# Unalome81/IEEE-802.11-OFDM-QPSK-Simulator

Measured on NVIDIA B200. Metric: OFDM symbols/s, TX+AWGN+RX chain (BER/EVM sweep), higher is better.
Workload: dtype f32+f64

## Files before the change

ieee-802.11-ofdm-qpsk-simulator_b200/csrc/ofdm_b200.cu:

```cuda
#include <cmath>
#include <cstdio>
#include <cstdlib>
#include <cstring>
#include <mutex>
#include <new>
#include <set>
#include <utility>

#include "ofdm_chain.cuh"
#include "ofdm_stream.cuh"
#include "ofdm_mc_quad.cuh"
#include "ofdm_sweep.cuh"

using namespace ofdm;

struct ofdm_ctx {
    int device = 0;
    int sm_count = 0;
    cudaStream_t stream = nullptr;
    bool owns_stream = false;
    cudaStream_t copy_stream = nullptr;
    cudaEvent_t copy_done[2] = {nullptr, nullptr}, call_start = nullptr;
    uint64_t launches = 0;
    bool force_generic = false;
// ... 21 lines not shown

const signed char kLk[53] = {1, 1, -1, -1, 1, 1, -1, 1, -1, 1, 1, 1, 1, 1, 1, -1, -1, 1, 1, -1, 1, -1, 1, 1, 1, 1, 0,
                             1, -1, -1, 1, 1, -1, 1, -1, 1, -1, -1, -1, -1, -1, 1, 1, -1, -1, 1, -1, 1, -1, 1, 1, 1, 1};

int fail(ofdm_ctx *ctx, int status, const char *what, cudaError_t e = cudaSuccess)
{
    if (ctx) {
        if (e != cudaSuccess) snprintf(ctx->err, sizeof ctx->err, "%s: %s", what, cudaGetErrorString(e));
        else snprintf(ctx->err, sizeof ctx->err, "%s", what);
    }
    return status;
}

#define OFDM_CUDA(ctx, call)                                                   \
    do {                                                                       \
        cudaError_t e_ = (call);                                               \
        if (e_ != cudaSuccess) return fail((ctx), OFDM_ERR_CUDA, #call, e_);   \
    } while (0)

#define OFDM_REQUIRE(ctx, cond)                                                          \
    do {                                                                                 \
        if (!(cond)) return fail((ctx), OFDM_ERR_INVALID, "invalid argument: " #cond);   \
    } while (0)

int check_launch(ofdm_ctx *ctx, const char *name)
{
    cudaError_t e = cudaGetLastError();
    if (e != cudaSuccess) return fail(ctx, OFDM_ERR_CUDA, name, e);
    ctx->launches += 1;
    return OFDM_OK;
}

int bind(ofdm_ctx *ctx)
{
    if (!ctx) return OFDM_ERR_INVALID;
    OFDM_CUDA(ctx, cudaSetDevice(ctx->device));
    return OFDM_OK;
}

template <typename K>
cudaError_t allow_smem(ofdm_ctx *ctx, K kernel, size_t bytes)
{
    static std::mutex mu;
    static std::set<std::pair<const void *, int>> done;
    std::lock_guard<std::mutex> lock(mu);
    const std::pair<const void *, int> key(reinterpret_cast<const void *>(kernel), ctx->device);
    if (done.count(key)) return cudaSuccess;
    const cudaError_t e = cudaFuncSetAttribute(kernel, cudaFuncAttributeMaxDynamicSharedMemorySize, (int)bytes);
    if (e == cudaSuccess) done.insert(key);
    return e;
}

template <typename K>
int grid_for(ofdm_ctx *ctx, K kernel, size_t dyn_smem, long work_items_per_block_iter, long work)
{
    int per_sm = 1;
    if (cudaOccupancyMaxActiveBlocksPerMultiprocessor(&per_sm, kernel, kThreads, dyn_smem) != cudaSuccess || per_sm < 1) per_sm = 1;
    long full = (long)per_sm * ctx->sm_count;
    long need = (work + work_items_per_block_iter - 1) / work_items_per_block_iter;
    long g = need < full ? need : full;
    return (int)(g < 1 ? 1 : g);
}

int stream_grid(ofdm_ctx *ctx, long rows, int rows_per_block, int per_sm)
{
    const long need = (rows + rows_per_block - 1) / rows_per_block, full = (long)per_sm * ctx->sm_count;
    const long g = need < full ? need : full;
    return (int)(g < 1 ? 1 : g);
}

int ensure_scratch(ofdm_ctx *ctx, int slot, size_t bytes, void **out)
{
    if (ctx->scratch_bytes[slot] < bytes) {
        if (ctx->scratch[slot]) { cudaFree(ctx->scratch[slot]); ctx->scratch[slot] = nullptr; ctx->scratch_bytes[slot] = 0; }
        cudaError_t e = cudaMalloc(&ctx->scratch[slot], bytes);
        if (e != cudaSuccess) return fail(ctx, OFDM_ERR_NOMEM, "cudaMalloc(scratch)", e);
        ctx->scratch_bytes[slot] = bytes;
    }
    *out = ctx->scratch[slot];
    return OFDM_OK;
}

float snr_linear(float snr_db)
{
    return (float)pow(10.0, (double)(snr_db / 10));
}

__global__ void k_power_prefix(const float2 *__restrict__ x, int n, float *__restrict__ out)
{
    float p = 0.f;
    for (int i = 0; i < n; ++i) {
        const double h = hypot_glibc((double)x[i].x, (double)x[i].y);
        p = __double2float_rn(__dadd_rn((double)p, __dmul_rn(h, h)));
    }
    *out = p;
}

struct DeviceTables {
    bool ready = false;
    float lts_freq[128], lts_time[320], sts_time[320], lts_power_prefix;
};
std::mutex g_tables_mutex;
DeviceTables g_tables[64];

int upload_tables(ofdm_ctx *ctx, const float *lts_time , float power_prefix)
{
    Tables t;
    memset(&t, 0, sizeof t);
    for (int k = 0; k < 32; ++k) t.tw64[k] = make_double2(kTw64[k][0], kTw64[k][1]);
    for (int k = 0; k < 64; ++k) {
// ... 783 lines not shown
    if (int st = ensure_scratch(ctx, 2, (size_t)n_frames * sizeof(float), &power)) return st;
    if (int st = ensure_scratch(ctx, 3, sizeof(ofdm_counters) * (size_t)n_snr, &cnt)) return st;
    if (!ctx->copy_stream) {
        OFDM_CUDA(ctx, cudaStreamCreateWithFlags(&ctx->copy_stream, cudaStreamNonBlocking));
        for (int i = 0; i < 2; ++i) OFDM_CUDA(ctx, cudaEventCreateWithFlags(&ctx->copy_done[i], cudaEventDisableTiming));
        OFDM_CUDA(ctx, cudaEventCreateWithFlags(&ctx->call_start, cudaEventDisableTiming));
    }
    OFDM_CUDA(ctx, cudaEventRecord(ctx->call_start, ctx->stream));
    OFDM_CUDA(ctx, cudaStreamWaitEvent(ctx->copy_stream, ctx->call_start, 0));
    OFDM_CUDA(ctx, cudaMemsetAsync(cnt, 0, sizeof(ofdm_counters) * (size_t)n_snr, ctx->stream));
    const long chunk = 65536;
    int c = 0;
    for (long f0 = 0; f0 < n_frames; f0 += chunk, ++c) {
        const long n = n_frames - f0 < chunk ? n_frames - f0 : chunk;
        char *db = (char *)bits + f0 * bits_per_frame, *dg = (char *)g + f0 * g_per_frame;
        OFDM_CUDA(ctx, cudaMemcpyAsync(db, (const char *)bits_host + f0 * bits_per_frame, n * bits_per_frame, cudaMemcpyHostToDevice, ctx->copy_stream));
        const char *hg = (const char *)g_host + f0 * g_per_frame;
        if (n_sym <= 4) {
            OFDM_CUDA(ctx, cudaMemcpy2DAsync(dg + 32 * 4, g_per_frame, hg + 32 * 4, g_per_frame, 128 * 4, n, cudaMemcpyHostToDevice, ctx->copy_stream));
            for (int sy = 0; sy < n_sym; ++sy) {
                const size_t off = (size_t)(160 + 80 * sy + 16) * 4;
                OFDM_CUDA(ctx, cudaMemcpy2DAsync(dg + off, g_per_frame, hg + off, g_per_frame, 64 * 4, n, cudaMemcpyHostToDevice, ctx->copy_stream));
            }
        } else {
            OFDM_CUDA(ctx, cudaMemcpyAsync(dg, hg, n * g_per_frame, cudaMemcpyHostToDevice, ctx->copy_stream));
        }
        OFDM_CUDA(ctx, cudaEventRecord(ctx->copy_done[c & 1], ctx->copy_stream));
        OFDM_CUDA(ctx, cudaStreamWaitEvent(ctx->stream, ctx->copy_done[c & 1], 0));
        float *fr = (float *)frames + f0 * len * 2, *pw = (float *)power + f0;
        if (int st = ofdm_tx_frames(ctx, (const uint32_t *)db, fr, pw, n, n_sym, mode)) return st;
        if (int st = sweep_points(ctx, fr, (const float *)dg, pw, (const uint32_t *)db, n, n_sym, snr_db, n_snr, mode,
                                  (ofdm_counters *)cnt))
            return st;
    }
    OFDM_CUDA(ctx, cudaMemcpyAsync(out_host, cnt, sizeof(ofdm_counters) * (size_t)n_snr, cudaMemcpyDeviceToHost, ctx->stream));
    OFDM_CUDA(ctx, cudaStreamSynchronize(ctx->stream));
    return OFDM_OK;
}

}

namespace {
int sweep_points(ofdm_ctx *ctx, const float *frames, const float *g, const float *power, const uint32_t *bits, long n_frames, int n_sym,
                 const float *snr_db, int n_snr, int mode, ofdm_counters *counters)
{
    const bool aligned = ((uintptr_t)frames % 16 == 0) && ((uintptr_t)g % 16 == 0);
    const bool fused = ctx->fused_sweep && n_sym == 2 && aligned && !ctx->force_generic && !ctx->general_stream &&
                       (mode != OFDM_MODE_EXACT || ctx->checked);
    if (!fused) {
        for (int i = 0; i < n_snr; ++i)
            if (int st = ofdm_awgn_rx_inject(ctx, frames, g, power, bits, snr_db[i], n_frames, n_sym, mode, counters + i, nullptr)) return st;
        return OFDM_OK;
    }
    const size_t smem = sweep_smem_bytes();
    const long max_frames = 1L << 30;
    for (int s0 = 0; s0 < n_snr; s0 += kMaxSnr) {
        SweepParams p;
        memset(&p, 0, sizeof p);
        p.n_snr = n_snr - s0 < kMaxSnr ? n_snr - s0 : kMaxSnr;
        for (int i = 0; i < p.n_snr; ++i) p.snr_lin[i] = snr_linear(snr_db[s0 + i]);
        p.radius_scale = ctx->force_replay ? INFINITY : kRadius;
        p.replayed = ctx->replayed_dev;
        p.evm_guard = ctx->evm_guard;
        p.counters = counters + s0;
        for (long f0 = 0; f0 < n_frames; f0 += max_frames) {
            p.n_frames = n_frames - f0 < max_frames ? n_frames - f0 : max_frames;
            p.in = reinterpret_cast<const float2 *>(frames) + f0 * 320;
            p.g = g + f0 * 320;
            p.power = power + f0;
            p.tx_bits = bits + f0 * 6;
            auto launch = [&](auto k) -> int {
                OFDM_CUDA(ctx, allow_smem(ctx, k, smem));
                int grid = grid_for(ctx, k, smem, kWarpsPerBlock, p.n_frames);
                k<<<grid, kThreads, smem, ctx->stream>>>(p);
                return check_launch(ctx, "k_sweep_lin");
            };
            if (int st = mode == OFDM_MODE_EXACT ? launch(k_sweep_lin<kArithChecked>) : launch(k_sweep_lin<kArithFast>)) return st;
        }
    }
    return OFDM_OK;
}
}

extern "C" {

int ofdm_random_bits(ofdm_ctx *ctx, uint32_t seed, uint64_t frame0, long n_frames, int n_sym, uint32_t *bits)
{
    if (int st = bind(ctx)) return st;
    OFDM_REQUIRE(ctx, n_frames >= 0 && nsym_ok(n_sym));
    if (n_frames == 0) return OFDM_OK;
    OFDM_REQUIRE(ctx, bits != nullptr);
    long n = n_frames * n_sym;
    k_philox_bits<<<blocks_1d(n), 256, 0, ctx->stream>>>(seed, frame0, n, n_sym, bits);
    return check_launch(ctx, "k_philox_bits");
}

}

namespace {
int mc_awgn_core(ofdm_ctx *ctx, uint32_t seed, uint64_t frame0, long n_frames, int n_sym, const float *snr_db, const uint32_t *streams,
                 int n_snr, int mode, ofdm_counters *counters)
{
    if (n_sym == 2) {
        const size_t smem = mc_smem_bytes();
        const long max_frames = 1L << 30;
        for (long f0 = 0; f0 < n_frames; f0 += max_frames) {
            McParams p;
            memset(&p, 0, sizeof p);
            p.seed = seed; p.frame0 = frame0 + (uint64_t)f0; p.n_frames = n_frames - f0 < max_frames ? n_frames - f0 : max_frames;
            p.n_snr = n_snr; p.counters = counters;
            for (int i = 0; i < n_snr; ++i) {
                p.snr_lin[i] = snr_linear(snr_db[i]); p.inv_sqrt_snr[i] = (float)(1.0 / sqrt((double)p.snr_lin[i]));
                p.stream[i] = streams ? streams[i] : (uint32_t)i;
            }
            p.radius_scale = ctx->force_replay ? INFINITY : kRadius;
            p.replayed = ctx->replayed_dev;
            p.evm_guard = ctx->evm_guard;
            p.radius_chan = ctx->force_replay ? INFINITY : kChanRadius * sqrtf(320.f) * 1.001f;
            auto launch = [&](auto k) -> int {
                OFDM_CUDA(ctx, allow_smem(ctx, k, smem));
                int grid = grid_for(ctx, k, smem, kWarpsPerBlock, p.n_frames);
                k<<<grid, kThreads, smem, ctx->stream>>>(p);
                return check_launch(ctx, "k_mc_philox");
            };
            auto launch_quad = [&](auto k) -> int {
                const size_t qsmem = mc_quad_smem_bytes();
                OFDM_CUDA(ctx, allow_smem(ctx, k, qsmem));
// ... 521 lines not shown
```

ieee-802.11-ofdm-qpsk-simulator_b200/csrc/ofdm_chain.cuh:

```cuda
#pragma once
#include "ofdm_kernels.cuh"

namespace ofdm {

constexpr int kWin = 72;
constexpr int kMaxSnr = 64;
constexpr int kMaxTaps = 16;

struct ItemConst {
    int f_off[3];
    int bin[3];
    float sc[3];
    int word[3];
    int shift[3];
};

__constant__ unsigned char c_deal_bin[48] = { 2, 10, 12, 14, 16, 23, 49, 54,    1,  3, 18, 40, 46, 60, 61, 63,   22, 25, 45, 47, 48, 50, 52, 59,
                                              4,  6,  9, 11, 13, 24, 39, 58,    8, 41, 42, 44, 51, 53, 55, 62,    5, 15, 17, 19, 20, 26, 38, 56};

__device__ __forceinline__ ItemConst make_items(int lane)
{
    ItemConst c;
#pragma unroll
    for (int r = 0; r < 3; ++r) {
        const int sym = (lane >> 3) & 1;
        const int bin = c_deal_bin[(2 * r + (lane >> 4)) * 8 + (lane & 7)];
        const int d = c_tab.bin_data[bin];
        c.f_off[r] = sym * kWin + bin;
        c.bin[r] = bin;
        c.sc[r] = 0.5f * (float)c_tab.bin_lts[bin];
        c.word[r] = sym * 3 + (d >> 4);
        c.shift[r] = 2 * (d & 15);
    }
    return c;
}

template <bool EXACT>
__device__ __forceinline__ uint32_t item_eval(float2 F, float2 Hh, float sc, uint32_t txp, float &e2)
{
    return process_bin_hot<EXACT>(F, Hh, sc, txp, true, e2);
}

enum { kArithFast = 0, kArithExact = 1, kArithChecked = 2 };
constexpr float kRadius = 320.f * 5.9604645e-8f;
constexpr float kChanRadius = 18.f * 5.9604645e-8f;


__device__ __forceinline__ float window_radius(float2 n2v, float scale, float extra)
{
    float n2 = n2v.x + n2v.y;
    n2 += __shfl_xor_sync(0xffffffffu, n2, 1);
    n2 += __shfl_xor_sync(0xffffffffu, n2, 2);
    n2 += __shfl_xor_sync(0xffffffffu, n2, 4);
    float r;
    asm("sqrt.approx.ftz.f32 %0, %1;" : "=f"(r) : "f"(n2));
    return (n2 >= 1e-30f && n2 < 1e20f) ? fmaf(scale, r, extra) : __int_as_float(0x7f800000);
}

constexpr float kEvmGuard = 820.f;
template <int LEVEL, bool THR_GIVEN = false>
__device__ __forceinline__ uint32_t process_bin_spec(float2 F, float2 G, float k, uint32_t txp, float rF, float rH2, float den_min4,
                                                     float2 &e2, bool &doubt)
{
    const float a = F.x, b = F.y, c = G.x, d = G.y;
    const float2 pt = __fmul2_rn(make_float2(d, d), make_float2(b, a));
    const float2 S = __ffma2_rn(make_float2(c, c), F, make_float2(pt.x, -pt.y));
    const float sr = S.x, si = S.y;
    const float den = fmaf(c, c, d * d);
    float inv;
    asm("rcp.approx.ftz.f32 %0, %1;" : "=f"(inv) : "f"(den));
    const uint32_t sq = txp << 31, sx = (txp ^ (txp >> 1)) << 31;
    const uint32_t kb = __float_as_uint(k);
    const uint32_t ei_ = (__float_as_uint(sr) ^ sx ^ kb) >> 31, eq_ = (__float_as_uint(si) ^ sq ^ kb) >> 31;
    bool safe;
    if (LEVEL >= 2) {
        float thr;
        if (THR_GIVEN) thr = rF;
        else {
            const float fa = fabsf(a) + fabsf(b), hc = fabsf(c) + fabsf(d);
            thr = fmaf(rF, hc + rH2, fmaf(rH2, fa, 1.2e-7f * (fa * hc)));
        }
        safe = (fminf(fabsf(sr), fabsf(si)) - thr) > 2e-30f && (THR_GIVEN || den < 1.6e14f) && den > den_min4;
    } else {
        safe = (THR_GIVEN || den < 1.6e14f) && den > den_min4;
    }
    doubt = doubt || !safe;
    const float2 U = __fmul2_rn(S, make_float2(inv, inv));
    const float2 D = __ffma2_rn(U, make_float2(k, k), make_float2(__uint_as_float(0xBF3504F3u ^ sx), __uint_as_float(0xBF3504F3u ^ sq)));
    e2 = __ffma2_rn(D, D, e2);
    return ei_ | (eq_ << 8) | ((ei_ & eq_) << 16);
}
__device__ __forceinline__ uint32_t process_bin_checked(float2 F, float2 G, float k, uint32_t txp, float rF, float rH2, float den_min4,
                                                        float2 &e2, bool &doubt)
{
    return process_bin_spec<2>(F, G, k, txp, rF, rH2, den_min4, e2, doubt);
}

struct McParams {
    uint32_t seed;
    uint64_t frame0;
    long n_frames;
    int n_snr;
    float snr_lin[kMaxSnr];
    float inv_sqrt_snr[kMaxSnr];
    uint32_t stream[kMaxSnr];
    float radius_scale;
    float radius_chan;
    float evm_guard;
    int n_taps;
    ofdm_counters *counters;
    unsigned long long *replayed;
};

struct WarpShared {
    float2 tile[kWarpTile];
    float2 lts[2][kWin];
    float2 body[2][kWin];
    uint2 res[kMaxSnr];
};

__device__ __noinline__ uint2 mc_point_replay(const float2 *src, double sigma_d, uint32_t seed, uint32_t stream, uint64_t fr,
                                              uint32_t txp3, float2 *ws_tile, float2 *ws_lts, unsigned long long *replayed)
{
    const int lane = threadIdx.x & 31, grp = lane >> 3, u = lane & 7;
    Tw<true> tw; tw.load(u);
    const ItemConst ic = make_items(lane);
    const int blk_base = (grp < 2 ? 8 + 16 * grp : 44 + 20 * (grp - 2)) + u;
    float za[4], zb[4];
    philox_normals4(seed, stream, fr, (uint32_t)blk_base, kDomainNoise, za);
    philox_normals4(seed, stream, fr, (uint32_t)(blk_base + 8), kDomainNoise, zb);
    float2 r[8];
#pragma unroll
    for (int i = 0; i < 8; ++i) {
        const int m = slot_m<true>(i);
        float2 s = src[u + 8 * m];
        s.x = add_noise<true>(s.x, m < 4 ? za[m & 3] : zb[m & 3], sigma_d, 0.f);
        r[i] = s;
    }
    fft64<true>(r, tw, ws_tile + grp * kGroupPitch, u);
    float2 *dst = grp < 2 ? ws_lts + grp * kWin : ws_tile + (grp - 2) * kWin;
#pragma unroll
    for (int j = 0; j < 8; ++j) dst[u + 8 * j] = r[j];
    __syncwarp();
// ... 1302 lines not shown
```

ieee-802.11-ofdm-qpsk-simulator_b200/csrc/ofdm_sweep.cuh:

```cuda
#pragma once
#include "ofdm_chain.cuh"

namespace ofdm {

struct SweepParams {
    const float2 *in;
    const float *g;
    const float *power;
    const uint32_t *tx_bits;
    long n_frames;
    int n_snr;
    float radius_scale;
    float evm_guard;
    float snr_lin[kMaxSnr];
    ofdm_counters *counters;
    unsigned long long *replayed;
};

struct alignas(16) SweepWarp {
    float2 tile[kWarpTile];
    float2 fx[4][kWin];
    float2 fn[4][kWin];
    StreamStage<true> st[kStages];
    uint64_t bar[kStages];
    float norm[8];
};
static_assert(sizeof(SweepWarp) % 16 == 0 && offsetof(SweepWarp, st) % 16 == 0 && offsetof(SweepWarp, norm) % 16 == 0, "SweepWarp alignment");

__device__ __forceinline__ float modulus_up(float2 z)
{
    float r;
    asm("sqrt.approx.ftz.f32 %0, %1;" : "=f"(r) : "f"(fmaf(z.x, z.x, z.y * z.y)));
    return fmaf(r, 1.000004f, 2e-19f);
}

template <int ARITH>
__global__ void __launch_bounds__(kThreads, 2) k_sweep_lin(SweepParams p)
{
    constexpr int LEVEL = ARITH == kArithChecked ? 2 : 1;
    extern __shared__ __align__(128) unsigned char s_raw[];
    const int lane = threadIdx.x & 31, warp = threadIdx.x >> 5, grp = lane >> 3, u = lane & 7;
    const int warp_u = __shfl_sync(0xffffffffu, warp, 0);
    SweepWarp &ws = reinterpret_cast<SweepWarp *>(s_raw)[warp];
    SweepWarp &ws_u = reinterpret_cast<SweepWarp *>(s_raw)[warp_u];
    float2 *tile = ws.tile + grp * kGroupPitch;
    Tw<false> tw; tw.load(u);
    const ItemConst ic = make_items(lane);
    const float k4[3] = {4.f * ic.sc[0], 4.f * ic.sc[1], 4.f * ic.sc[2]};
    constexpr int len = 320;
    const long stride = (long)gridDim.x * kWarpsPerBlock;
    const long f_first = (long)blockIdx.x * kWarpsPerBlock + warp_u;
    const double q = (double)kQpsk;
    const double ref2_frame = 96.0 * (2.0 * q * q);
    const float inv_ref2 = (float)(1.0 / ref2_frame);
    constexpr uint32_t kBytes = 4 * 512 + 4 * 256;

    const uint32_t stage0 = tma::saddr(&ws_u.st[0]);
    const uint32_t bar0 = tma::saddr(&ws_u.bar[0]);
    auto issue = [&](long f, int s) {
        if (tma::elect_one()) {
            const uint32_t bar = bar0 + 8u * (uint32_t)s;
            const uint32_t dst = stage0 + (uint32_t)s * (uint32_t)sizeof(StreamStage<true>);
            const char *x = reinterpret_cast<const char *>(p.in) + f * (len * 8);
            const char *g = reinterpret_cast<const char *>(p.g) + f * (len * 4);
            const uint32_t gd = dst + 4 * kWin * 8;
            tma::expect_tx_addr(bar, kBytes);
            tma::bulk_addr(dst + 0 * kWin * 8, x + 32 * 8, 512, bar);
            tma::bulk_addr(dst + 1 * kWin * 8, x + 96 * 8, 512, bar);
            tma::bulk_addr(dst + 2 * kWin * 8, x + 176 * 8, 512, bar);
            tma::bulk_addr(dst + 3 * kWin * 8, x + 256 * 8, 512, bar);
            tma::bulk_addr(gd + 0 * kWin * 4, g + 32 * 4, 256, bar);
            tma::bulk_addr(gd + 1 * kWin * 4, g + 96 * 4, 256, bar);
            tma::bulk_addr(gd + 2 * kWin * 4, g + 176 * 4, 256, bar);
            tma::bulk_addr(gd + 3 * kWin * 4, g + 256 * 4, 256, bar);
        }
    };
    if (lane == 0) {
        for (int s = 0; s < kStages; ++s) tma::mbar_init(&ws.bar[s], 1);
        tma::fence_mbar_init();
    }
    __syncwarp();
    for (int s = 0; s < kStages; ++s)
        if (f_first + s * stride < p.n_frames) issue(f_first + s * stride, s);

    uint32_t m_i[2] = {0, 0}, m_q[2] = {0, 0}, m_b[2] = {0, 0}, m_ferr[2] = {0, 0};
    float m_e2[2] = {0.f, 0.f}, m_evm[2] = {0.f, 0.f};
    double d_e2[2] = {0.0, 0.0}, d_evm[2] = {0.0, 0.0};
    uint32_t n_done = 0;
    uint32_t k = 0;
    for (long f = f_first; f < p.n_frames; f += stride, ++k) {
        const int s = (int)(k & 1u);
        const uint32_t phase = (k >> 1) & 1u;
        const float P = p.power[f];
        const uint32_t *wb = p.tx_bits + f * 6;
        uint32_t txw[3];
#pragma unroll
        for (int t = 0; t < 3; ++t) txw[t] = wb[ic.word[t]];

        tma::wait_addr(bar0 + 8u * (uint32_t)s, phase);
        float2 v[8];
        float gz[8];
        float2 n2x = make_float2(0.f, 0.f);
        float n2g = 0.f;
#pragma unroll
        for (int i = 0; i < 8; ++i) {
            v[i] = ws.st[s].x[grp][u + 8 * i];
            gz[i] = ws.st[s].g[grp][u + 8 * i];
            n2x = __ffma2_rn(v[i], v[i], n2x);
            n2g = fmaf(gz[i], gz[i], n2g);
        }
        __syncwarp();
        if (f + kStages * stride < p.n_frames) issue(f + kStages * stride, s);
        fft64<false>(v, tw, tile, u);
#pragma unroll
        for (int j = 0; j < 8; ++j) ws.fx[grp][u + 8 * j] = v[j];
#pragma unroll
        for (int i = 0; i < 8; ++i) v[i] = make_float2(gz[i], 0.f);
        fft64<false>(v, tw, tile, u);
#pragma unroll
        for (int j = 0; j < 8; ++j) ws.fn[grp][u + 8 * j] = v[j];
        float2 nn = make_float2(n2x.x + n2x.y, n2g);
#pragma unroll
        for (int o = 1; o < 8; o <<= 1)
            nn = __fadd2_rn(nn, make_float2(__shfl_xor_sync(0xffffffffu, nn.x, o), __shfl_xor_sync(0xffffffffu, nn.y, o)));
        {
            float rx, rn;
            asm("sqrt.approx.ftz.f32 %0, %1;" : "=f"(rx) : "f"(nn.x));
            asm("sqrt.approx.ftz.f32 %0, %1;" : "=f"(rn) : "f"(nn.y));
            const bool ok = nn.x >= 1e-30f && nn.x < 1e20f && nn.y < 1e20f;
            const float inf = __int_as_float(0x7f800000);
            if (u == 0) { ws.norm[grp] = ok ? p.radius_scale * rx : inf; ws.norm[4 + grp] = ok ? p.radius_scale * rn : inf; }
        }
        __syncwarp();
        const float4 rX = *reinterpret_cast<const float4 *>(ws.norm), rN = *reinterpret_cast<const float4 *>(ws.norm + 4);
        const float rHX = rX.x + rX.y, rHN = rN.x + rN.y;
        float2 FX[3], FN[3], GX[3], GN[3];
        float c0[3], c1[3], c2[3];
#pragma unroll
        for (int t = 0; t < 3; ++t) {
            const int bin = ic.bin[t];
            GX[t] = cadd(ws.fx[0][bin], ws.fx[1][bin]);
            GN[t] = cadd(ws.fn[0][bin], ws.fn[1][bin]);
            FX[t] = (&ws.fx[2][0])[ic.f_off[t]];
            FN[t] = (&ws.fn[2][0])[ic.f_off[t]];
            const bool sym0 = ic.f_off[t] < kWin;
            const float rFX = sym0 ? rX.z : rX.w, rFN = sym0 ? rN.z : rN.w;
            if (LEVEL >= 2) {
                const float faX = modulus_up(FX[t]), faN = modulus_up(FN[t]);
                const float hcX = modulus_up(GX[t]), hcN = modulus_up(GN[t]);
                const float A0 = hcX + rHX, A1 = hcN + rHN;
                c0[t] = fmaf(rFX, A0, fmaf(rHX, faX, 1.2e-7f * (faX * hcX)));
                c1[t] = fmaf(rFX, A1, fmaf(rFN, A0, fmaf(rHX, faN, fmaf(rHN, faX, 1.2e-7f * fmaf(faX, hcN, faN * hcX)))));
                c2[t] = fmaf(rFN, A1, fmaf(rHN, faN, 1.2e-7f * (faN * hcN)));
            } else { c0[t] = c1[t] = c2[t] = 0.f; }
        }
        __syncwarp();
#pragma unroll
        for (int t = 0; t < 3; ++t) {
            const uint32_t tp = txw[t] >> ic.shift[t];
            const uint32_t kb = __float_as_uint(k4[t]) & 0x80000000u;
            const uint32_t fq = (tp << 31) ^ kb, fi = ((tp ^ (tp >> 1)) << 31) ^ kb, gq = (tp >> 1) << 31;
            FX[t] = make_float2(__uint_as_float(__float_as_uint(FX[t].x) ^ fi), __uint_as_float(__float_as_uint(FX[t].y) ^ fq));
            FN[t] = make_float2(__uint_as_float(__float_as_uint(FN[t].x) ^ fi), __uint_as_float(__float_as_uint(FN[t].y) ^ fq));
            GX[t].y = __uint_as_float(__float_as_uint(GX[t].y) ^ gq);
            GN[t].y = __uint_as_float(__float_as_uint(GN[t].y) ^ gq);
        }
        float sig_lo = 0.f, sig_hi = 0.f;
        if (lane < p.n_snr) sig_lo = __fsqrt_rn(__fdiv_rn(P, p.snr_lin[lane]));
        if (p.n_snr > 32 && lane + 32 < p.n_snr) sig_hi = __fsqrt_rn(__fdiv_rn(P, p.snr_lin[lane + 32]));
        float *sigs = reinterpret_cast<float *>(&ws.fn[1][0]);
        sigs[lane] = sig_lo; sigs[lane + 32] = sig_hi;
        if (lane < 2) sigs[64 + lane] = 0.f;
        __syncwarp();

        uint2 *res = reinterpret_cast<uint2 *>(&ws.fn[0][0]);
        const float g2_limit = p.radius_scale * 1.58e6f;
        struct PointState { float sg, rH2, den_min4; float2 e2v; uint32_t pk; bool doubt; };
        auto point_begin = [&](float sg) {
            PointState q;
            q.sg = sg;
            q.rH2 = fmaf(sg, rHN, rHX);
            const float gd = p.evm_guard * q.rH2;
            q.den_min4 = gd * gd;
            q.e2v = make_float2(0.f, 0.f);
            q.pk = 0; q.doubt = !(q.rH2 < g2_limit);
            return q;
        };
        auto point_item = [&](PointState &q, int t) {
            const float2 sg2 = make_float2(q.sg, q.sg);
            const float2 F = __ffma2_rn(sg2, FN[t], FX[t]);
            const float2 G = __ffma2_rn(sg2, GN[t], GX[t]);
            const float thr = fmaf(fmaf(c2[t], q.sg, c1[t]), q.sg, c0[t]);
            q.pk += process_bin_spec<LEVEL, true>(F, G, 2.f, 0u, thr, q.rH2, q.den_min4, q.e2v, q.doubt);
        };
        auto resolve_point = [&](int si, float sg, uint32_t &pk, float &e2) {
            bool replay = true;
            if (LEVEL >= 2) {
                const float4 qX = *reinterpret_cast<const float4 *>(ws.norm), qN = *reinterpret_cast<const float4 *>(ws.norm + 4);
                const float2 sg2 = make_float2(sg, sg);
                const float rH2 = fmaf(sg, rHN, rHX);
                const float gd = p.evm_guard * rH2, den_min4 = gd * gd;
                bool doubt2 = false;
                float2 e2w = make_float2(0.f, 0.f);
                uint32_t pk2 = 0;
#pragma unroll
                for (int t = 0; t < 3; ++t) {
                    const float2 F = __ffma2_rn(sg2, FN[t], FX[t]);
                    const float2 G = __ffma2_rn(sg2, GN[t], GX[t]);
                    const bool sym0 = ic.f_off[t] < kWin;
                    const float rF = fmaf(sg, sym0 ? qN.z : qN.w, sym0 ? qX.z : qX.w);
                    const float fa = modulus_up(F), hc = modulus_up(G);
                    const float thr = fmaf(rF, hc + rH2, fmaf(rH2, fa, 1.2e-7f * (fa * hc)));
                    pk2 += process_bin_spec<LEVEL, true>(F, G, 2.f, 0u, thr, rH2, den_min4, e2w, doubt2);
                }
                replay = __any_sync(0xffffffffu, doubt2);
            }
            if (replay) {
                const double sigma_d = __dsqrt_rn((double)__fdiv_rn(P, p.snr_lin[si]));
                const uint2 r = stream_frame_replay<kNoiseInject>(p.in + f * len, p.g + f * len, wb, sigma_d, 0u, 0u, 0ull,
                                                                  ws.tile, &ws.fx[0][0], p.replayed);
                pk = r.x; e2 = __uint_as_float(r.y);
            }
        };
        uint32_t pk_raw0 = 0, pk_raw1 = 0;
        float2 e2_pend = make_float2(0.f, 0.f);
        constexpr int kStep = LEVEL >= 2 ? 2 : 1;
        float2 red = make_float2(0.f, 0.f), red_in = red;
        constexpr bool kSpread = LEVEL < 2;
        auto red_issue = [&](int o, float after) {
            const int m = kSpread ? o | (int)(__float_as_uint(after) & 0x80000000u) : o;
            red_in = make_float2(__shfl_xor_sync(0xffffffffu, red.x, m), __shfl_xor_sync(0xffffffffu, red.y, m));
        };
        auto red_take = [&]() { red = __fadd2_rn(red, red_in); };
        for (int si = 0; si < p.n_snr; si += kStep) {
            const uint32_t pk_sum0 = __reduce_add_sync(0xffffffffu, pk_raw0);
            const uint32_t pk_sum1 = kStep == 2 ? __reduce_add_sync(0xffffffffu, pk_raw1) : 0u;
            red = e2_pend;
            red_issue(16, 0.f);
            const bool two = kStep == 2 && si + 1 < p.n_snr;
            const int sj = two ? si + 1 : si;
            float sg0, sg1;
            if (kStep == 2) { const float2 sp = *reinterpret_cast<const float2 *>(sigs + si); sg0 = sp.x; sg1 = sp.y; }
            else { sg0 = sigs[si]; sg1 = 0.f; }
            PointState q0 = point_begin(sg0), q1 = point_begin(sg1);
            point_item(q0, 0); red_take(); red_issue(8, q0.e2v.x);
            point_item(q0, 1); red_take(); red_issue(4, q0.e2v.x);
            point_item(q0, 2); red_take(); red_issue(2, q0.e2v.x);
            if (kStep == 2) {
                point_item(q1, 0); red_take(); red_issue(1, q1.e2v.x);
                point_item(q1, 1); red_take();
            } else {
                red_take(); red_issue(1, 0.f); red_take();
            }
            if (lane == 0 && si > 0) {
                res[si - kStep] = make_uint2(pk_sum0, __float_as_uint(red.x));
                if (kStep == 2) res[si - 1] = make_uint2(pk_sum1, __float_as_uint(red.y));
            }
            if (kStep == 2) point_item(q1, 2);
            uint32_t pk0 = q0.pk, pk1 = q1.pk;
            float e20 = q0.e2v.x + q0.e2v.y, e21 = q1.e2v.x + q1.e2v.y;
            if (__any_sync(0xffffffffu, q0.doubt || (kStep == 2 && q1.doubt))) {
                if (__any_sync(0xffffffffu, q0.doubt)) resolve_point(si, sg0, pk0, e20);
                if (two && __any_sync(0xffffffffu, q1.doubt)) resolve_point(sj, sg1, pk1, e21);
            }
            pk_raw0 = pk0; pk_raw1 = pk1;
            e2_pend = make_float2(e20, e21);
        }
        {
            const uint32_t pk_sum0 = __reduce_add_sync(0xffffffffu, pk_raw0);
            const uint32_t pk_sum1 = kStep == 2 ? __reduce_add_sync(0xffffffffu, pk_raw1) : 0u;
            float2 r = e2_pend;
#pragma unroll
            for (int o = 16; o > 0; o >>= 1)
                r = __fadd2_rn(r, make_float2(__shfl_xor_sync(0xffffffffu, r.x, o), __shfl_xor_sync(0xffffffffu, r.y, o)));
            const int last = (p.n_snr - 1) & ~(kStep - 1);
            if (lane == 0) {
                res[last] = make_uint2(pk_sum0, __float_as_uint(r.x));
                if (last + 1 < p.n_snr) res[last + 1] = make_uint2(pk_sum1, __float_as_uint(r.y));
            }
        }
        __syncwarp();
#pragma unroll
        for (int h = 0; h < 2; ++h) {
            if (h == 1 && p.n_snr <= 32) break;
            const uint2 r = res[lane + 32 * h];
            const bool mine = lane + 32 * h < p.n_snr;
            const uint32_t pk = mine ? r.x : 0u;
            const float e2 = mine ? __uint_as_float(r.y) : 0.f;
            float evm;
            asm("sqrt.approx.ftz.f32 %0, %1;" : "=f"(evm) : "f"(e2 * inv_ref2));
            m_i[h] += pk & 0xFFu; m_q[h] += (pk >> 8) & 0xFFu; m_b[h] += pk >> 16; m_ferr[h] += pk != 0u;
            m_e2[h] += e2; m_evm[h] += evm;
        }
        n_done += 1;
        if ((n_done & 63u) == 0u) {
#pragma unroll
            for (int h = 0; h < 2; ++h) { d_e2[h] += (double)m_e2[h]; d_evm[h] += (double)m_evm[h]; m_e2[h] = 0.f; m_evm[h] = 0.f; }
        }
    }
    if (n_done == 0) return;
#pragma unroll
    for (int h = 0; h < 2; ++h) {
        const int si = lane + 32 * h;
        if (si >= p.n_snr) continue;
        ofdm_counters *o = p.counters + si;
        const unsigned long long ti = m_i[h], tq = m_q[h], tb = m_b[h];
        atomicAdd(reinterpret_cast<unsigned long long *>(&o->bit_errors), ti + 2ull * tq - 2ull * tb);
        atomicAdd(reinterpret_cast<unsigned long long *>(&o->rail_errors), ti + tq);
        atomicAdd(reinterpret_cast<unsigned long long *>(&o->frames_in_error), (unsigned long long)m_ferr[h]);
        atomicAdd(reinterpret_cast<unsigned long long *>(&o->frames), (unsigned long long)n_done);
        atomicAdd(reinterpret_cast<unsigned long long *>(&o->bits), 192ull * n_done);
        atomicAdd(&o->sum_err2, d_e2[h] + (double)m_e2[h]);
        atomicAdd(&o->sum_ref2, ref2_frame * (double)n_done);
        atomicAdd(&o->sum_evm_lin, d_evm[h] + (double)m_evm[h]);
    }
}

inline size_t sweep_smem_bytes() { return sizeof(SweepWarp) * kWarpsPerBlock; }

}
```

Baseline: 9.476 billion.

## Share channel estimate across symbol pairs and process three SNR points per step

Remaps the sweep kernel's per-lane subcarrier items so that two of each lane's three items share one data bin across both symbols. The channel value G, its squared magnitude and its approximate reciprocal are then computed once and reused for the second symbol through a sign flip. The SNR loop now handles three points per iteration in both arithmetic modes, with interleaved shuffle reductions. Doubtful points are recorded in a bitmask and resolved after the loop instead of inline, so the main loop stays branch-light. The cost is higher register pressure, a padded sigma layout in shared memory, and a more intricate, less obviously correct replay and reduction path.

```diff
diff --git a/ieee-802.11-ofdm-qpsk-simulator_b200/csrc/ofdm_b200.cu b/ieee-802.11-ofdm-qpsk-simulator_b200/csrc/ofdm_b200.cu
--- a/ieee-802.11-ofdm-qpsk-simulator_b200/csrc/ofdm_b200.cu
+++ b/ieee-802.11-ofdm-qpsk-simulator_b200/csrc/ofdm_b200.cu
@@ -97,10 +97,10 @@
 }
 
 template <typename K>
-int grid_for(ofdm_ctx *ctx, K kernel, size_t dyn_smem, long work_items_per_block_iter, long work)
+int grid_for(ofdm_ctx *ctx, K kernel, size_t dyn_smem, long work_items_per_block_iter, long work, int threads = kThreads)
 {
     int per_sm = 1;
-    if (cudaOccupancyMaxActiveBlocksPerMultiprocessor(&per_sm, kernel, kThreads, dyn_smem) != cudaSuccess || per_sm < 1) per_sm = 1;
+    if (cudaOccupancyMaxActiveBlocksPerMultiprocessor(&per_sm, kernel, threads, dyn_smem) != cudaSuccess || per_sm < 1) per_sm = 1;
     long full = (long)per_sm * ctx->sm_count;
     long need = (work + work_items_per_block_iter - 1) / work_items_per_block_iter;
     long g = need < full ? need : full;
@@ -990,7 +990,6 @@
             if (int st = ofdm_awgn_rx_inject(ctx, frames, g, power, bits, snr_db[i], n_frames, n_sym, mode, counters + i, nullptr)) return st;
         return OFDM_OK;
     }
-    const size_t smem = sweep_smem_bytes();
     const long max_frames = 1L << 30;
     for (int s0 = 0; s0 < n_snr; s0 += kMaxSnr) {
         SweepParams p;
@@ -1008,9 +1007,11 @@
             p.power = power + f0;
             p.tx_bits = bits + f0 * 6;
             auto launch = [&](auto k) -> int {
+                constexpr int warps = kSweepWarps;
+                const size_t smem = sweep_smem_bytes(warps);
                 OFDM_CUDA(ctx, allow_smem(ctx, k, smem));
-                int grid = grid_for(ctx, k, smem, kWarpsPerBlock, p.n_frames);
-                k<<<grid, kThreads, smem, ctx->stream>>>(p);
+                const int grid = grid_for(ctx, k, smem, warps, p.n_frames, warps * 32);
+                k<<<grid, warps * 32, smem, ctx->stream>>>(p);
                 return check_launch(ctx, "k_sweep_lin");
             };
             if (int st = mode == OFDM_MODE_EXACT ? launch(k_sweep_lin<kArithChecked>) : launch(k_sweep_lin<kArithFast>)) return st;
diff --git a/ieee-802.11-ofdm-qpsk-simulator_b200/csrc/ofdm_chain.cuh b/ieee-802.11-ofdm-qpsk-simulator_b200/csrc/ofdm_chain.cuh
--- a/ieee-802.11-ofdm-qpsk-simulator_b200/csrc/ofdm_chain.cuh
+++ b/ieee-802.11-ofdm-qpsk-simulator_b200/csrc/ofdm_chain.cuh
@@ -59,16 +59,13 @@
 
 constexpr float kEvmGuard = 820.f;
 template <int LEVEL, bool THR_GIVEN = false>
-__device__ __forceinline__ uint32_t process_bin_spec(float2 F, float2 G, float k, uint32_t txp, float rF, float rH2, float den_min4,
-                                                     float2 &e2, bool &doubt)
+__device__ __forceinline__ uint32_t process_bin_spec_den(float2 F, float2 G, float den, float inv, float k, uint32_t txp, float rF,
+                                                         float rH2, float den_min4, float2 &e2, bool &doubt)
 {
     const float a = F.x, b = F.y, c = G.x, d = G.y;
     const float2 pt = __fmul2_rn(make_float2(d, d), make_float2(b, a));
     const float2 S = __ffma2_rn(make_float2(c, c), F, make_float2(pt.x, -pt.y));
     const float sr = S.x, si = S.y;
-    const float den = fmaf(c, c, d * d);
-    float inv;
-    asm("rcp.approx.ftz.f32 %0, %1;" : "=f"(inv) : "f"(den));
     const uint32_t sq = txp << 31, sx = (txp ^ (txp >> 1)) << 31;
     const uint32_t kb = __float_as_uint(k);
     const uint32_t ei_ = (__float_as_uint(sr) ^ sx ^ kb) >> 31, eq_ = (__float_as_uint(si) ^ sq ^ kb) >> 31;
@@ -89,6 +86,15 @@
     const float2 D = __ffma2_rn(U, make_float2(k, k), make_float2(__uint_as_float(0xBF3504F3u ^ sx), __uint_as_float(0xBF3504F3u ^ sq)));
     e2 = __ffma2_rn(D, D, e2);
     return ei_ | (eq_ << 8) | ((ei_ & eq_) << 16);
+}
+template <int LEVEL, bool THR_GIVEN = false>
+__device__ __forceinline__ uint32_t process_bin_spec(float2 F, float2 G, float k, uint32_t txp, float rF, float rH2, float den_min4,
+                                                     float2 &e2, bool &doubt)
+{
+    const float den = fmaf(G.x, G.x, G.y * G.y);
+    float inv;
+    asm("rcp.approx.ftz.f32 %0, %1;" : "=f"(inv) : "f"(den));
+    return process_bin_spec_den<LEVEL, THR_GIVEN>(F, G, den, inv, k, txp, rF, rH2, den_min4, e2, doubt);
 }
 __device__ __forceinline__ uint32_t process_bin_checked(float2 F, float2 G, float k, uint32_t txp, float rF, float rH2, float den_min4,
                                                         float2 &e2, bool &doubt)
diff --git a/ieee-802.11-ofdm-qpsk-simulator_b200/csrc/ofdm_sweep.cuh b/ieee-802.11-ofdm-qpsk-simulator_b200/csrc/ofdm_sweep.cuh
--- a/ieee-802.11-ofdm-qpsk-simulator_b200/csrc/ofdm_sweep.cuh
+++ b/ieee-802.11-ofdm-qpsk-simulator_b200/csrc/ofdm_sweep.cuh
@@ -34,10 +34,42 @@
     return fmaf(r, 1.000004f, 2e-19f);
 }
 
+__constant__ unsigned char c_sweep_pair[32] = { 1,  2,  5,  8, 11, 16, 19, 41, 44, 45, 46, 52, 54, 55, 58, 63,
+                                                3,  4, 10, 12, 17, 18, 22, 23, 25, 47, 48, 53, 56, 59, 61, 62};
+__constant__ unsigned char c_sweep_single[16] = { 6, 14, 15, 20, 26, 40, 49, 50,    9, 13, 24, 38, 39, 42, 51, 60};
+
+struct SweepItems {
+    int bin[2];
+    int f_off[3];
+    float k4[3];
+    int word[3];
+    int shift[3];
+};
+
+__device__ __forceinline__ SweepItems make_sweep_items(int lane)
+{
+    SweepItems c;
+    c.bin[0] = c_sweep_pair[lane];
+    c.bin[1] = c_sweep_single[(lane >> 4) * 8 + (lane & 7)];
+#pragma unroll
+    for (int t = 0; t < 3; ++t) {
+        const int bin = c.bin[t >> 1], sym = t == 2 ? (lane >> 3) & 1 : t;
+        const int d = c_tab.bin_data[bin];
+        c.f_off[t] = sym * kWin + bin;
+        c.k4[t] = 4.f * (0.5f * (float)c_tab.bin_lts[bin]);
+        c.word[t] = sym * 3 + (d >> 4);
+        c.shift[t] = 2 * (d & 15);
+    }
+    return c;
+}
+
+constexpr int kSweepWarps = 6;
+
 template <int ARITH>
-__global__ void __launch_bounds__(kThreads, 2) k_sweep_lin(SweepParams p)
+__global__ void __launch_bounds__(kSweepWarps * 32, 2) k_sweep_lin(SweepParams p)
 {
     constexpr int LEVEL = ARITH == kArithChecked ? 2 : 1;
+    constexpr int kWarps = kSweepWarps;
     extern __shared__ __align__(128) unsigned char s_raw[];
     const int lane = threadIdx.x & 31, warp = threadIdx.x >> 5, grp = lane >> 3, u = lane & 7;
     const int warp_u = __shfl_sync(0xffffffffu, warp, 0);
@@ -45,15 +77,15 @@
     SweepWarp &ws_u = reinterpret_cast<SweepWarp *>(s_raw)[warp_u];
     float2 *tile = ws.tile + grp * kGroupPitch;
     Tw<false> tw; tw.load(u);
-    const ItemConst ic = make_items(lane);
-    const float k4[3] = {4.f * ic.sc[0], 4.f * ic.sc[1], 4.f * ic.sc[2]};
+    const SweepItems ic = make_sweep_items(lane);
     constexpr int len = 320;
-    const long stride = (long)gridDim.x * kWarpsPerBlock;
-    const long f_first = (long)blockIdx.x * kWarpsPerBlock + warp_u;
+    const long stride = (long)gridDim.x * kWarps;
+    const long f_first = (long)blockIdx.x * kWarps + warp_u;
     const double q = (double)kQpsk;
     const double ref2_frame = 96.0 * (2.0 * q * q);
     const float inv_ref2 = (float)(1.0 / ref2_frame);
     constexpr uint32_t kBytes = 4 * 512 + 4 * 256;
+    constexpr int kStep = 3;
 
     const uint32_t stage0 = tma::saddr(&ws_u.st[0]);
     const uint32_t bar0 = tma::saddr(&ws_u.bar[0]);
@@ -134,48 +166,59 @@
         __syncwarp();
         const float4 rX = *reinterpret_cast<const float4 *>(ws.norm), rN = *reinterpret_cast<const float4 *>(ws.norm + 4);
         const float rHX = rX.x + rX.y, rHN = rN.x + rN.y;
-        float2 FX[3], FN[3], GX[3], GN[3];
-        float c0[3], c1[3], c2[3];
+        float2 FX[3], FN[3], GX[2], GN[2];
+        float c0[3], c1[3], c2[3], hcX[2], hcN[2];
+#pragma unroll
+        for (int e = 0; e < 2; ++e) {
+            const int bin = ic.bin[e];
+            GX[e] = cadd(ws.fx[0][bin], ws.fx[1][bin]);
+            GN[e] = cadd(ws.fn[0][bin], ws.fn[1][bin]);
+            if (LEVEL >= 2) { hcX[e] = modulus_up(GX[e]); hcN[e] = modulus_up(GN[e]); }
+        }
 #pragma unroll
         for (int t = 0; t < 3; ++t) {
-            const int bin = ic.bin[t];
-            GX[t] = cadd(ws.fx[0][bin], ws.fx[1][bin]);
-            GN[t] = cadd(ws.fn[0][bin], ws.fn[1][bin]);
             FX[t] = (&ws.fx[2][0])[ic.f_off[t]];
             FN[t] = (&ws.fn[2][0])[ic.f_off[t]];
             const bool sym0 = ic.f_off[t] < kWin;
             const float rFX = sym0 ? rX.z : rX.w, rFN = sym0 ? rN.z : rN.w;
             if (LEVEL >= 2) {
                 const float faX = modulus_up(FX[t]), faN = modulus_up(FN[t]);
-                const float hcX = modulus_up(GX[t]), hcN = modulus_up(GN[t]);
-                const float A0 = hcX + rHX, A1 = hcN + rHN;
-                c0[t] = fmaf(rFX, A0, fmaf(rHX, faX, 1.2e-7f * (faX * hcX)));
-                c1[t] = fmaf(rFX, A1, fmaf(rFN, A0, fmaf(rHX, faN, fmaf(rHN, faX, 1.2e-7f * fmaf(faX, hcN, faN * hcX)))));
-                c2[t] = fmaf(rFN, A1, fmaf(rHN, faN, 1.2e-7f * (faN * hcN)));
+                const float hX = hcX[t >> 1], hN = hcN[t >> 1];
+                const float A0 = hX + rHX, A1 = hN + rHN;
+                c0[t] = fmaf(rFX, A0, fmaf(rHX, faX, 1.2e-7f * (faX * hX)));
+                c1[t] = fmaf(rFX, A1, fmaf(rFN, A0, fmaf(rHX, faN, fmaf(rHN, faX, 1.2e-7f * fmaf(faX, hN, faN * hX)))));
+                c2[t] = fmaf(rFN, A1, fmaf(rHN, faN, 1.2e-7f * (faN * hN)));
             } else { c0[t] = c1[t] = c2[t] = 0.f; }
         }
         __syncwarp();
+        uint32_t gq[3];
 #pragma unroll
         for (int t = 0; t < 3; ++t) {
             const uint32_t tp = txw[t] >> ic.shift[t];
-            const uint32_t kb = __float_as_uint(k4[t]) & 0x80000000u;
-            const uint32_t fq = (tp << 31) ^ kb, fi = ((tp ^ (tp >> 1)) << 31) ^ kb, gq = (tp >> 1) << 31;
+            const uint32_t kb = __float_as_uint(ic.k4[t]) & 0x80000000u;
+            const uint32_t fq = (tp << 31) ^ kb, fi = ((tp ^ (tp >> 1)) << 31) ^ kb;
+            gq[t] = (tp >> 1) << 31;
             FX[t] = make_float2(__uint_as_float(__float_as_uint(FX[t].x) ^ fi), __uint_as_float(__float_as_uint(FX[t].y) ^ fq));
             FN[t] = make_float2(__uint_as_float(__float_as_uint(FN[t].x) ^ fi), __uint_as_float(__float_as_uint(FN[t].y) ^ fq));
-            GX[t].y = __uint_as_float(__float_as_uint(GX[t].y) ^ gq);
-            GN[t].y = __uint_as_float(__float_as_uint(GN[t].y) ^ gq);
-        }
+        }
+#pragma unroll
+        for (int e = 0; e < 2; ++e) {
+            GX[e].y = __uint_as_float(__float_as_uint(GX[e].y) ^ gq[2 * e]);
+            GN[e].y = __uint_as_float(__float_as_uint(GN[e].y) ^ gq[2 * e]);
+        }
+        const uint32_t g_rel = gq[0] ^ gq[1];
         float sig_lo = 0.f, sig_hi = 0.f;
         if (lane < p.n_snr) sig_lo = __fsqrt_rn(__fdiv_rn(P, p.snr_lin[lane]));
         if (p.n_snr > 32 && lane + 32 < p.n_snr) sig_hi = __fsqrt_rn(__fdiv_rn(P, p.snr_lin[lane + 32]));
+        auto sig_pos = [](int i) { return (i / 3) * 4 + i % 3; };
         float *sigs = reinterpret_cast<float *>(&ws.fn[1][0]);
-        sigs[lane] = sig_lo; sigs[lane + 32] = sig_hi;
-        if (lane < 2) sigs[64 + lane] = 0.f;
+        sigs[sig_pos(lane)] = sig_lo; sigs[sig_pos(lane + 32)] = sig_hi;
+        if (lane < 2) sigs[sig_pos(64 + lane)] = 0.f;
         __syncwarp();
 
         uint2 *res = reinterpret_cast<uint2 *>(&ws.fn[0][0]);
         const float g2_limit = p.radius_scale * 1.58e6f;
-        struct PointState { float sg, rH2, den_min4; float2 e2v; uint32_t pk; bool doubt; };
+        struct PointState { float sg, rH2, den_min4; float2 e2v; uint32_t pk; bool doubt; float2 G; float den, inv; };
         auto point_begin = [&](float sg) {
             PointState q;
             q.sg = sg;
@@ -188,95 +231,112 @@
         };
         auto point_item = [&](PointState &q, int t) {
             const float2 sg2 = make_float2(q.sg, q.sg);
+            if (t != 1) {
+                q.G = __ffma2_rn(sg2, GN[t >> 1], GX[t >> 1]);
+                q.den = fmaf(q.G.x, q.G.x, q.G.y * q.G.y);
+                asm("rcp.approx.ftz.f32 %0, %1;" : "=f"(q.inv) : "f"(q.den));
+            }
+            const float2 G = t == 1 ? make_float2(q.G.x, __uint_as_float(__float_as_uint(q.G.y) ^ g_rel)) : q.G;
             const float2 F = __ffma2_rn(sg2, FN[t], FX[t]);
-            const float2 G = __ffma2_rn(sg2, GN[t], GX[t]);
             const float thr = fmaf(fmaf(c2[t], q.sg, c1[t]), q.sg, c0[t]);
-            q.pk += process_bin_spec<LEVEL, true>(F, G, 2.f, 0u, thr, q.rH2, q.den_min4, q.e2v, q.doubt);
+            q.pk += process_bin_spec_den<LEVEL, true>(F, G, q.den, q.inv, 2.f, 0u, thr, q.rH2, q.den_min4, q.e2v, q.doubt);
         };
-        auto resolve_point = [&](int si, float sg, uint32_t &pk, float &e2) {
-            bool replay = true;
-            if (LEVEL >= 2) {
-                const float4 qX = *reinterpret_cast<const float4 *>(ws.norm), qN = *reinterpret_cast<const float4 *>(ws.norm + 4);
-                const float2 sg2 = make_float2(sg, sg);
-                const float rH2 = fmaf(sg, rHN, rHX);
-                const float gd = p.evm_guard * rH2, den_min4 = gd * gd;
-                bool doubt2 = false;
-                float2 e2w = make_float2(0.f, 0.f);
-                uint32_t pk2 = 0;
-#pragma unroll
-                for (int t = 0; t < 3; ++t) {
-                    const float2 F = __ffma2_rn(sg2, FN[t], FX[t]);
-                    const float2 G = __ffma2_rn(sg2, GN[t], GX[t]);
-                    const bool sym0 = ic.f_off[t] < kWin;
-                    const float rF = fmaf(sg, sym0 ? qN.z : qN.w, sym0 ? qX.z : qX.w);
-                    const float fa = modulus_up(F), hc = modulus_up(G);
-                    const float thr = fmaf(rF, hc + rH2, fmaf(rH2, fa, 1.2e-7f * (fa * hc)));
-                    pk2 += process_bin_spec<LEVEL, true>(F, G, 2.f, 0u, thr, rH2, den_min4, e2w, doubt2);
+        uint32_t pk_raw[kStep];
+        float e2_pend[kStep], red[kStep], red_in[kStep];
+#pragma unroll
+        for (int j = 0; j < kStep; ++j) { pk_raw[j] = 0; e2_pend[j] = 0.f; }
+        auto red_issue = [&](int o) {
+#pragma unroll
+            for (int j = 0; j < kStep; ++j) red_in[j] = __shfl_xor_sync(0xffffffffu, red[j], o);
+        };
+        auto red_take = [&]() {
+#pragma unroll
+            for (int j = 0; j < kStep; ++j) red[j] += red_in[j];
+        };
+        uint64_t doubt_mask = 0;
+        for (int si = 0, sk = 0; si < p.n_snr; si += kStep, sk += 4) {
+            uint32_t pk_sum[kStep];
+#pragma unroll
+            for (int j = 0; j < kStep; ++j) { pk_sum[j] = __reduce_add_sync(0xffffffffu, pk_raw[j]); red[j] = e2_pend[j]; }
+            red_issue(16);
+            PointState q[kStep];
+            const float4 sp = *reinterpret_cast<const float4 *>(sigs + sk);
+            q[0] = point_begin(sp.x); q[1] = point_begin(sp.y); q[2] = point_begin(sp.z);
+#pragma unroll
+            for (int t = 0; t < 3; ++t) {
+#pragma unroll
+                for (int j = 0; j < kStep; ++j) {
+                    const int n = t * kStep + j;
+                    point_item(q[j], t);
+                    if (n < 4) { red_take(); red_issue(8 >> n); }
+                    else if (n == 4) red_take();
                 }
-                replay = __any_sync(0xffffffffu, doubt2);
-            }
-            if (replay) {
-                const double sigma_d = __dsqrt_rn((double)__fdiv_rn(P, p.snr_lin[si]));
-                const uint2 r = stream_frame_replay<kNoiseInject>(p.in + f * len, p.g + f * len, wb, sigma_d, 0u, 0u, 0ull,
-                                                                  ws.tile, &ws.fx[0][0], p.replayed);
-                pk = r.x; e2 = __uint_as_float(r.y);
-            }
-        };
-        uint32_t pk_raw0 = 0, pk_raw1 = 0;
-        float2 e2_pend = make_float2(0.f, 0.f);
-        constexpr int kStep = LEVEL >= 2 ? 2 : 1;
-        float2 red = make_float2(0.f, 0.f), red_in = red;
-        constexpr bool kSpread = LEVEL < 2;
-        auto red_issue = [&](int o, float after) {
-            const int m = kSpread ? o | (int)(__float_as_uint(after) & 0x80000000u) : o;
-            red_in = make_float2(__shfl_xor_sync(0xffffffffu, red.x, m), __shfl_xor_sync(0xffffffffu, red.y, m));
-        };
-        auto red_take = [&]() { red = __fadd2_rn(red, red_in); };
-        for (int si = 0; si < p.n_snr; si += kStep) {
-            const uint32_t pk_sum0 = __reduce_add_sync(0xffffffffu, pk_raw0);
-            const uint32_t pk_sum1 = kStep == 2 ? __reduce_add_sync(0xffffffffu, pk_raw1) : 0u;
-            red = e2_pend;
-            red_issue(16, 0.f);
-            const bool two = kStep == 2 && si + 1 < p.n_snr;
-            const int sj = two ? si + 1 : si;
-            float sg0, sg1;
-            if (kStep == 2) { const float2 sp = *reinterpret_cast<const float2 *>(sigs + si); sg0 = sp.x; sg1 = sp.y; }
-            else { sg0 = sigs[si]; sg1 = 0.f; }
-            PointState q0 = point_begin(sg0), q1 = point_begin(sg1);
-            point_item(q0, 0); red_take(); red_issue(8, q0.e2v.x);
-            point_item(q0, 1); red_take(); red_issue(4, q0.e2v.x);
-            point_item(q0, 2); red_take(); red_issue(2, q0.e2v.x);
-            if (kStep == 2) {
-                point_item(q1, 0); red_take(); red_issue(1, q1.e2v.x);
-                point_item(q1, 1); red_take();
-            } else {
-                red_take(); red_issue(1, 0.f); red_take();
             }
             if (lane == 0 && si > 0) {
-                res[si - kStep] = make_uint2(pk_sum0, __float_as_uint(red.x));
-                if (kStep == 2) res[si - 1] = make_uint2(pk_sum1, __float_as_uint(red.y));
-            }
-            if (kStep == 2) point_item(q1, 2);
-            uint32_t pk0 = q0.pk, pk1 = q1.pk;
-            float e20 = q0.e2v.x + q0.e2v.y, e21 = q1.e2v.x + q1.e2v.y;
-            if (__any_sync(0xffffffffu, q0.doubt || (kStep == 2 && q1.doubt))) {
-                if (__any_sync(0xffffffffu, q0.doubt)) resolve_point(si, sg0, pk0, e20);
-                if (two && __any_sync(0xffffffffu, q1.doubt)) resolve_point(sj, sg1, pk1, e21);
-            }
-            pk_raw0 = pk0; pk_raw1 = pk1;
-            e2_pend = make_float2(e20, e21);
+#pragma unroll
+                for (int j = 0; j < kStep; ++j) res[si - kStep + j] = make_uint2(pk_sum[j], __float_as_uint(red[j]));
+            }
+            uint32_t bits = 0;
+#pragma unroll
+            for (int j = 0; j < kStep; ++j) {
+                pk_raw[j] = q[j].pk;
+                e2_pend[j] = q[j].e2v.x + q[j].e2v.y;
+                bits |= (uint32_t)q[j].doubt << j;
+            }
+            doubt_mask |= (uint64_t)bits << si;
         }
         {
-            const uint32_t pk_sum0 = __reduce_add_sync(0xffffffffu, pk_raw0);
-            const uint32_t pk_sum1 = kStep == 2 ? __reduce_add_sync(0xffffffffu, pk_raw1) : 0u;
-            float2 r = e2_pend;
-#pragma unroll
-            for (int o = 16; o > 0; o >>= 1)
-                r = __fadd2_rn(r, make_float2(__shfl_xor_sync(0xffffffffu, r.x, o), __shfl_xor_sync(0xffffffffu, r.y, o)));
-            const int last = (p.n_snr - 1) & ~(kStep - 1);
-            if (lane == 0) {
-                res[last] = make_uint2(pk_sum0, __float_as_uint(r.x));
-                if (last + 1 < p.n_snr) res[last + 1] = make_uint2(pk_sum1, __float_as_uint(r.y));
+            const int last = (p.n_snr - 1) / kStep * kStep;
+#pragma unroll
+            for (int j = 0; j < kStep; ++j) {
+                const uint32_t pk_sum = __reduce_add_sync(0xffffffffu, pk_raw[j]);
+                float r = e2_pend[j];
+#pragma unroll
+                for (int o = 16; o > 0; o >>= 1) r += __shfl_xor_sync(0xffffffffu, r, o);
+                if (lane == 0) res[last + j] = make_uint2(pk_sum, __float_as_uint(r));
+            }
+        }
+        {
+            if (p.n_snr < 64) doubt_mask &= (1ull << p.n_snr) - 1ull;
+            uint64_t todo = __reduce_or_sync(0xffffffffu, (uint32_t)doubt_mask);
+            if (p.n_snr > 32) todo |= (uint64_t)__reduce_or_sync(0xffffffffu, (uint32_t)(doubt_mask >> 32)) << 32;
+            __syncwarp();
+            while (todo != 0) {
+                const int si = __ffsll((long long)todo) - 1;
+                todo &= todo - 1;
+                const float sg = sigs[sig_pos(si)];
+                bool replay = true;
+                if (LEVEL >= 2) {
+                    const float4 qX = *reinterpret_cast<const float4 *>(ws.norm), qN = *reinterpret_cast<const float4 *>(ws.norm + 4);
+                    const float2 sg2 = make_float2(sg, sg);
+                    const float rH2 = fmaf(sg, rHN, rHX);
+                    const float gd = p.evm_guard * rH2, den_min4 = gd * gd;
+                    bool doubt2 = false;
+                    float2 e2w = make_float2(0.f, 0.f);
+                    float2 G;
+#pragma unroll
+                    for (int t = 0; t < 3; ++t) {
+                        if (t != 1) G = __ffma2_rn(sg2, GN[t >> 1], GX[t >> 1]);
+                        const float2 Gt = t == 1 ? make_float2(G.x, __uint_as_float(__float_as_uint(G.y) ^ g_rel)) : G;
+                        const float2 F = __ffma2_rn(sg2, FN[t], FX[t]);
+                        const bool sym0 = ic.f_off[t] < kWin;
+                        const float rF = fmaf(sg, sym0 ? qN.z : qN.w, sym0 ? qX.z : qX.w);
+                        const float fa = modulus_up(F), hc = modulus_up(Gt);
+                        const float thr = fmaf(rF, hc + rH2, fmaf(rH2, fa, 1.2e-7f * (fa * hc)));
+                        process_bin_spec<LEVEL, true>(F, Gt, 2.f, 0u, thr, rH2, den_min4, e2w, doubt2);
+                    }
+                    replay = __any_sync(0xffffffffu, doubt2);
+                }
+                if (replay) {
+                    const double sigma_d = __dsqrt_rn((double)__fdiv_rn(P, p.snr_lin[si]));
+                    const uint2 r = stream_frame_replay<kNoiseInject>(p.in + f * len, p.g + f * len, wb, sigma_d, 0u, 0u, 0ull,
+                                                                      ws.tile, &ws.fx[0][0], p.replayed);
+                    const uint32_t pk_sum = __reduce_add_sync(0xffffffffu, r.x);
+                    float e2 = __uint_as_float(r.y);
+#pragma unroll
+                    for (int o = 16; o > 0; o >>= 1) e2 += __shfl_xor_sync(0xffffffffu, e2, o);
+                    if (lane == 0) res[si] = make_uint2(pk_sum, __float_as_uint(e2));
+                }
             }
         }
         __syncwarp();
@@ -316,6 +376,6 @@
     }
 }
 
-inline size_t sweep_smem_bytes() { return sizeof(SweepWarp) * kWarpsPerBlock; }
+inline size_t sweep_smem_bytes(int warps) { return sizeof(SweepWarp) * warps; }
 
 }
```

New measurement: 10.62 billion (median of 6 runs). +12.1%, better.
